# thanosDelatolas/eva-vos

Measured on AMD Instinct MI355X. Metric: frames/sec STCN mask-propagate 480p 1-obj, higher is better.
Workload: dtype f32; 1 GPU; DAVIS-17-val-shaped 480x854 (padded 480x864) single-object STCN propagate: fresh engine, interact(mask,0), T=66 frames/video, mem_freq=5, top_k=50; one video per step per GPU; videos_per_gpu=38, streams_per_gpu=4, key_lookahead=0, clips=8 distinct synthetic clips (one per pooled engine), weights=synthetic recipe seed 0 (no checkpoints offline)

## Files before the change

### eva_vos_amd/csrc/winograd4.hip

```cpp
#include <hip/hip_ext.h>

#include <cstdio>
#include <cstdlib>
#include <type_traits>

#include "wino_common.h"

namespace stcn {

typedef float f32x4 __attribute__((ext_vector_type(4)));
typedef float f32x16 __attribute__((ext_vector_type(16)));

#ifdef STCN_W4_CLOCK
__device__ unsigned long long g_w4_clock[2 * 8192];
#if STCN_W4_CLOCK == 2
#define W4_MFMA(a_, b_, c_) w4_fake_mfma(a_, b_, c_)
#endif
#endif
#ifndef W4_MFMA
#define W4_MFMA(a_, b_, c_) __builtin_amdgcn_mfma_f32_32x32x2f32(a_, b_, c_, 0, 0, 0)
#endif

static constexpr int W4T = 32;
static constexpr int W4N = 32;
static constexpr int W4W = 12;

#if defined(STCN_W4_CLOCK) && STCN_W4_CLOCK == 2
__device__ __forceinline__ f32x16 w4_fake_mfma(float a, float b, f32x16 c) {
#pragma unroll
    for (int e = 0; e < 16; ++e) asm volatile("v_fma_f32 %0, %1, %2, %0" : "+v"(c[e]) : "v"(a), "v"(b));
    return c;
}
#endif

__device__ __forceinline__ void bt6(const f32x4 &d0, const f32x4 &d1, const f32x4 &d2, const f32x4 &d3, const f32x4 &d4, const f32x4 &d5,
                                    f32x4 &o0, f32x4 &o1, f32x4 &o2, f32x4 &o3, f32x4 &o4, f32x4 &o5) {
    o0 = d0 * 1.265625f - d2 * 2.8125f + d4;
    const f32x4 e1 = d4 - d2 * 2.25f, f1 = d3 * 0.75f - d1 * 1.6875f;
    o1 = e1 + f1;
    o2 = e1 - f1;
    const f32x4 e2 = d4 - d2 * 0.5625f, f2 = d3 * 1.5f - d1 * 0.84375f;
    o3 = e2 + f2;
    o4 = e2 - f2;
    o5 = d1 * 1.265625f - d3 * 2.8125f + d5;
}

__global__ __launch_bounds__(256) void wino4_input_kernel(const float *__restrict__ x, unsigned x_bytes, long x_bs, int H, int W, int C,
                                                          int relu_in, int TH, int TW, int Mt, int Mt_pad, int cb_per_chunk,
                                                          int tile_lo, int tile_hi, float *__restrict__ V) {
    const long i = xcd_contiguous_block((int)blockIdx.x, (int)gridDim.x) * 256L + threadIdx.x;
    const int c16 = (int)(i & 7);
    const long tile = tile_lo + (i >> 3);
    if (tile >= tile_hi) return;
    const int KB = C / 8, NCB = C / 32;
    const int cb0 = blockIdx.y * cb_per_chunk, cb1 = min(NCB, cb0 + cb_per_chunk);
    const bool live = tile < Mt;
    const int tpi = TH * TW;
    const int b = live ? (int)(tile / tpi) : 0;
    const int r = live ? (int)(tile - (long)b * tpi) : 0;
    const int ty = r / TW, tx = r - ty * TW;
    const int y0 = 4 * ty - 1, x0 = 4 * tx - 1;
    unsigned long long ok = 0;
#pragma unroll
    for (int yy = 0; yy < 6; ++yy)
#pragma unroll
        for (int xx = 0; xx < 6; ++xx)
            if (live && (unsigned)(y0 + yy) < (unsigned)H && (unsigned)(x0 + xx) < (unsigned)W) ok |= 1ull << (yy * 6 + xx);
    const __amdgpu_buffer_rsrc_t rx = __builtin_amdgcn_make_buffer_rsrc(const_cast<float *>(x), 0, x_bytes, 0x00020000);
    const int xoff = (int)((b * x_bs + ((long)y0 * W + x0) * C + 4 * c16) * 4);
    const long ps = ((long)KB * Mt_pad) << 3;
    const float lo = relu_in ? 0.f : -__builtin_inff();
    for (int cb = cb0; cb < cb1; ++cb) {
        f32x4 t[6][6];
#pragma unroll
        for (int xx = 0; xx < 6; ++xx) {
            f32x4 d[6];
#pragma unroll
            for (int yy = 0; yy < 6; ++yy) {
                const unsigned vo = ((ok >> (yy * 6 + xx)) & 1ull) ? (unsigned)(xoff + ((yy * W + xx) * C + 32 * cb) * 4) : 0x80000000u;
                f32x4 v = __builtin_bit_cast(f32x4, __builtin_amdgcn_raw_buffer_load_b128(rx, vo, 0, 0));
                v.x = fmaxf(v.x, lo); v.y = fmaxf(v.y, lo); v.z = fmaxf(v.z, lo); v.w = fmaxf(v.w, lo);
                d[yy] = v;
            }
            bt6(d[0], d[1], d[2], d[3], d[4], d[5], t[0][xx], t[1][xx], t[2][xx], t[3][xx], t[4][xx], t[5][xx]);
        }
        const int kb = cb * 4 + (c16 >> 1);
        float *base = V + (((long)kb * Mt_pad + tile) << 3) + 4 * (c16 & 1);
#pragma unroll
        for (int xi = 0; xi < 6; ++xi) {
            f32x4 v[6];
            bt6(t[xi][0], t[xi][1], t[xi][2], t[xi][3], t[xi][4], t[xi][5], v[0], v[1], v[2], v[3], v[4], v[5]);
            float *dst = base + (long)(xi * 6) * ps;
#pragma unroll
            for (int nu = 0; nu < 6; ++nu) *reinterpret_cast<f32x4 *>(dst + nu * ps) = v[nu];
        }
    }
}

struct Wino4G {
    const float *V, *U;
    unsigned v_bytes, u_bytes;
    int Mt, Mt_pad, KB, N;
    int TH, TW, OH, OW, B, M;
    const float *bias, *res;
    long res_bs; int res_bmod;
    float *y; long y_bs;
    int relu_out;
    FastDiv fd_tpi, fd_tw, fd_tiles_n;
    int full_wg, pieces, kb_per_piece;
    float *partial;
    int tm0;
    int xb_m, xb_n, xb_cols;
};

template <int MB>
__global__ __launch_bounds__(64 * W4W) void wino4_gemm_kernel(const Wino4G p, const int tiles_n) {
    constexpr int PPW = 3, WT = W4T * MB;
    extern __shared__ __attribute__((aligned(16))) float smem[];
    int swz, piece = -1, kb0 = 0, kb1 = p.KB;
    if (MB == 1 && p.pieces > 1 && (int)blockIdx.x >= p.full_wg) {
        const int j = xcd_contiguous_block((int)blockIdx.x - p.full_wg, (int)gridDim.x - p.full_wg);
        const int rt = j / p.pieces;
        piece = j - rt * p.pieces;
        swz = p.full_wg + rt;
        kb0 = piece * p.kb_per_piece;
        kb1 = min(p.KB, kb0 + p.kb_per_piece);
    } else {
        swz = xcd_contiguous_block((int)blockIdx.x, MB == 1 && p.pieces > 1 ? p.full_wg : (int)gridDim.x);
    }
    int tm_l = fastdiv(swz, p.fd_tiles_n), tn = swz - tm_l * tiles_n;
    if (p.xb_m > 0 && piece < 0) {
        const int per = p.xb_m * p.xb_n, blk = swz / per, in = swz - blk * per;
        const int bm_i = blk / p.xb_cols, bn_i = blk - bm_i * p.xb_cols, im = in / p.xb_n;
        tm_l = bm_i * p.xb_m + im;
        tn = bn_i * p.xb_n + (in - im * p.xb_n);
    }
    const int tm = tm_l + p.tm0;
    const int t = threadIdx.x, lane = t & 63, l31 = lane & 31, h = lane >> 5;
    const int wave = __builtin_amdgcn_readfirstlane(t >> 6);
    const int pos0 = PPW * wave;

    const __amdgpu_buffer_rsrc_t rv = __builtin_amdgcn_make_buffer_rsrc(const_cast<float *>(p.V), 0, p.v_bytes, 0x00020000);
    const __amdgpu_buffer_rsrc_t ru = __builtin_amdgcn_make_buffer_rsrc(const_cast<float *>(p.U), 0, p.u_bytes, 0x00020000);
    const unsigned vl = (unsigned)(l31 * 32 + h * 16);
    unsigned sa0[PPW], sb0[PPW];
#pragma unroll
    for (int pi = 0; pi < PPW; ++pi) {
        sa0[pi] = (unsigned)((((long)(pos0 + pi) * p.KB + kb0) * p.Mt_pad + tm * WT) * 32);
        sb0[pi] = (unsigned)((((long)(pos0 + pi) * p.KB + kb0) * p.N + tn * W4N) * 32);
    }
    const unsigned sa = (unsigned)p.Mt_pad * 32u, sb = (unsigned)p.N * 32u;

    f32x16 acc[PPW][MB];
#pragma unroll
    for (int pi = 0; pi < PPW; ++pi)
#pragma unroll
        for (int bi = 0; bi < MB; ++bi)
#pragma unroll
            for (int e = 0; e < 16; ++e) acc[pi][bi][e] = 0.f;

    const int nk = kb1 - kb0;
    auto load1 = [&](int k, int pi, f32x4 (&fa)[MB], f32x4 &fb) {
        const unsigned oa = sa0[pi] + (unsigned)k * sa, ob = sb0[pi] + (unsigned)k * sb;
#pragma unroll
        for (int bi = 0; bi < MB; ++bi) fa[bi] = __builtin_bit_cast(f32x4, __builtin_amdgcn_raw_buffer_load_b128(rv, vl, oa + bi * 1024u, 0));
        fb = __builtin_bit_cast(f32x4, __builtin_amdgcn_raw_buffer_load_b128(ru, vl, ob, 0));
    };
    auto compute1 = [&](int pi, const f32x4 (&fa)[MB], const f32x4 &fb) {
#pragma unroll
        for (int j = 0; j < 4; ++j)
#pragma unroll
            for (int bi = 0; bi < MB; ++bi) acc[pi][bi] = W4_MFMA(fa[bi][j], fb[j], acc[pi][bi]);
    };
#ifdef STCN_W4_CLOCK
    unsigned long long ck_t0 = 0, ck_r0 = 0;
    if (wave == 0) {
        __builtin_amdgcn_sched_barrier(0);
        ck_t0 = __builtin_amdgcn_s_memtime();
        ck_r0 = __builtin_amdgcn_s_memrealtime();
        __builtin_amdgcn_s_waitcnt(0xC07F);
        __builtin_amdgcn_sched_barrier(0);
    }
#endif
    if (MB == 1) {
        f32x4 fa[3][PPW][MB], fb[3][PPW];
        auto load = [&](int k, int set) {
#pragma unroll
            for (int pi = 0; pi < PPW; ++pi) load1(k, pi, fa[set][pi], fb[set][pi]);
        };
        auto compute = [&](int set) {
#pragma unroll
            for (int j = 0; j < 4; ++j)
#pragma unroll
                for (int pi = 0; pi < PPW; ++pi)
#pragma unroll
                    for (int bi = 0; bi < MB; ++bi)
                        acc[pi][bi] = W4_MFMA(fa[set][pi][bi][j], fb[set][pi][j], acc[pi][bi]);
        };
        load(0, 0);
        load(min(1, nk - 1), 1);
        int k = 0;
        for (; k + 2 < nk; k += 3) {
            load(k + 2, 2);
            __builtin_amdgcn_sched_barrier(0);
            compute(0);
            __builtin_amdgcn_sched_barrier(0);
            load(min(k + 3, nk - 1), 0);
            __builtin_amdgcn_sched_barrier(0);
            compute(1);
            __builtin_amdgcn_sched_barrier(0);
            load(min(k + 4, nk - 1), 1);
            __builtin_amdgcn_sched_barrier(0);
            compute(2);
            __builtin_amdgcn_sched_barrier(0);
        }
        if (k < nk) compute(0);
        if (k + 1 < nk) compute(1);
    } else {
        f32x4 fa[2][PPW], fb[2][PPW];
        auto loadA = [&](int k, int bi, f32x4 (&d)[PPW]) {
#pragma unroll
            for (int pi = 0; pi < PPW; ++pi)
                d[pi] = __builtin_bit_cast(f32x4, __builtin_amdgcn_raw_buffer_load_b128(rv, vl, sa0[pi] + (unsigned)k * sa + bi * 1024u, 0));
        };
        auto loadB = [&](int k, f32x4 (&d)[PPW]) {
#pragma unroll
            for (int pi = 0; pi < PPW; ++pi)
                d[pi] = __builtin_bit_cast(f32x4, __builtin_amdgcn_raw_buffer_load_b128(ru, vl, sb0[pi] + (unsigned)k * sb, 0));
        };
        auto comp = [&](int bi, const f32x4 (&a)[PPW], const f32x4 (&bb)[PPW]) {
#pragma unroll
            for (int j = 0; j < 4; ++j)
#pragma unroll
                for (int pi = 0; pi < PPW; ++pi) acc[pi][bi] = W4_MFMA(a[pi][j], bb[pi][j], acc[pi][bi]);
        };
        loadB(0, fb[0]);
        loadA(0, 0, fa[0]);
        for (int k = 0; k < nk; k += 2) {
            const int k2 = min(k + 2, nk - 2);
            loadA(k, 1, fa[1]);
            __builtin_amdgcn_sched_barrier(0);
            comp(0, fa[0], fb[0]);
            __builtin_amdgcn_sched_barrier(0);
            loadB(k + 1, fb[1]);
            loadA(k + 1, 0, fa[0]);
            __builtin_amdgcn_sched_barrier(0);
            comp(1, fa[1], fb[0]);
            __builtin_amdgcn_sched_barrier(0);
            loadA(k + 1, 1, fa[1]);
            __builtin_amdgcn_sched_barrier(0);
            comp(0, fa[0], fb[1]);
            __builtin_amdgcn_sched_barrier(0);
            loadB(k2, fb[0]);
            loadA(k2, 0, fa[0]);
            __builtin_amdgcn_sched_barrier(0);
            comp(1, fa[1], fb[1]);
            __builtin_amdgcn_sched_barrier(0);
        }
    }
#ifdef STCN_W4_CLOCK
    if (wave == 0) {
        __builtin_amdgcn_sched_barrier(0);
        const unsigned long long ck_t1 = __builtin_amdgcn_s_memtime(), ck_r1 = __builtin_amdgcn_s_memrealtime();
        __builtin_amdgcn_s_waitcnt(0xC07F);
        __builtin_amdgcn_sched_barrier(0);
        if (lane == 0 && blockIdx.x < 8192) { g_w4_clock[2 * blockIdx.x] = ck_t1 - ck_t0; g_w4_clock[2 * blockIdx.x + 1] = ck_r1 - ck_r0; }
    }
#endif
    const int chq = t & 7, tl = (t >> 3) & 31;
    const int jh = __builtin_amdgcn_readfirstlane(t >> 8);
    const int tpi = p.TH * p.TW, ohw = p.OH * p.OW;
    const int n = tn * W4N + 4 * chq;
    const bool kpiece = MB == 1 && piece >= 0;
    const float lo = p.relu_out ? 0.f : -__builtin_inff();
    const __amdgpu_buffer_rsrc_t rres = __builtin_amdgcn_make_buffer_rsrc(const_cast<float *>(p.res ? p.res : p.y), 0, -1, 0x00020000);
    const __amdgpu_buffer_rsrc_t ry = __builtin_amdgcn_make_buffer_rsrc(p.y, 0, -1, 0x00020000);
    const unsigned y_bs = (unsigned)(p.y_bs ? p.y_bs : (long)ohw * p.N);
#pragma unroll
    for (int half = 0; half < MB; ++half) {
        int toff = 32 * half + tl;
        asm volatile("" : "+v"(toff));
        const long gt = (long)tm * WT + toff;
        const bool work = jh < 2 && gt < p.Mt;
        const int gtc = (int)min(gt, (long)p.Mt - 1);
        const int b = fastdiv(gtc, p.fd_tpi);
        const int rr = gtc - b * tpi;
        const int ty = fastdiv(rr, p.fd_tw), tx = rr - ty * p.TW;
        unsigned prow[4], pcol[2];
#pragma unroll
        for (int i2 = 0; i2 < 4; ++i2) prow[i2] = (unsigned)(min(4 * ty + i2, p.OH - 1) * p.OW * p.N) * 4u;
#pragma unroll
        for (int j = 0; j < 2; ++j) pcol[j] = (unsigned)(min(4 * tx + 2 * jh + j, p.OW - 1) * p.N + n) * 4u;
        if (half) __syncthreads();
#pragma unroll
        for (int pi = 0; pi < PPW; ++pi)
#pragma unroll
            for (int r = 0; r < 16; ++r)
                smem[((pos0 + pi) * W4T + (r & 3) + 8 * (r >> 2) + 4 * h) * W4N + l31] = acc[pi][half][r];
        f32x4 yv[2][4], bv = {0.f, 0.f, 0.f, 0.f};
        if (p.bias && !kpiece) {
            int nb = n;
            asm volatile("" : "+v"(nb));
            bv = *reinterpret_cast<const f32x4 *>(p.bias + nb);
        }
        if (p.res && !kpiece && jh < 2) {
            const unsigned rb = (unsigned)(p.res_bmod ? b % p.res_bmod : b) * (unsigned)p.res_bs * 4u;
#pragma unroll
            for (int j = 0; j < 2; ++j)
#pragma unroll
                for (int i2 = 0; i2 < 4; ++i2)
                    yv[j][i2] = __builtin_bit_cast(f32x4, __builtin_amdgcn_raw_buffer_load_b128(rres, rb + prow[i2] + pcol[j], 0, 0));
        } else {
#pragma unroll
            for (int j = 0; j < 2; ++j)
#pragma unroll
                for (int i2 = 0; i2 < 4; ++i2) yv[j][i2] = f32x4{0.f, 0.f, 0.f, 0.f};
        }
        __syncthreads();
        if (!work) continue;
        auto zrow = [&](int xi, auto JH, f32x4 (&zr)[2]) {
            f32x4 m[6];
            int ro4 = (xi * 6 * W4T + tl) * (W4N / 4) + chq;
            asm volatile("" : "+v"(ro4));
#pragma unroll
            for (int nu = 0; nu < 6; ++nu) m[nu] = reinterpret_cast<const f32x4 *>(smem)[ro4 + nu * W4T * (W4N / 4)];
            if (decltype(JH)::value == 0) {
                zr[0] = m[0] + (m[1] + m[2]) + (m[3] + m[4]);
                zr[1] = (m[1] - m[2]) * 0.75f + (m[3] - m[4]) * 1.5f;
            } else {
                zr[0] = (m[1] + m[2]) * 0.5625f + (m[3] + m[4]) * 2.25f;
                zr[1] = (m[1] - m[2]) * 0.421875f + (m[3] - m[4]) * 3.375f + m[5];
            }
        };
        auto columns = [&](auto JH) {
            f32x4 za[2];
#pragma unroll
            for (int j = 0; j < 2; ++j)
#pragma unroll
                for (int i2 = 0; i2 < 4; ++i2) yv[j][i2] += bv;
            zrow(0, JH, za);
#pragma unroll
            for (int j = 0; j < 2; ++j) yv[j][0] += za[j];
            constexpr float c1[4] = {0.75f, -0.75f, 1.5f, -1.5f}, c2[4] = {0.5625f, 0.5625f, 2.25f, 2.25f},
                            c3[4] = {0.421875f, -0.421875f, 3.375f, -3.375f};
#pragma unroll
            for (int xi = 1; xi < 5; ++xi) {
                __builtin_amdgcn_sched_barrier(0);
                zrow(xi, JH, za);
#pragma unroll
                for (int j = 0; j < 2; ++j) {
                    yv[j][0] += za[j];
                    yv[j][1] += za[j] * c1[xi - 1];
                    yv[j][2] += za[j] * c2[xi - 1];
                    yv[j][3] += za[j] * c3[xi - 1];
                }
            }
            __builtin_amdgcn_sched_barrier(0);
            zrow(5, JH, za);
#pragma unroll
            for (int j = 0; j < 2; ++j) yv[j][3] += za[j];
        };
        if (jh == 0) columns(std::integral_constant<int, 0>{});
        else columns(std::integral_constant<int, 1>{});
        if (kpiece) {
            float *dst = p.partial + (((long)(swz - p.full_wg) * p.pieces + piece) * W4T + tl) * (16 * W4N) + 4 * chq;
#pragma unroll
            for (int j = 0; j < 2; ++j)
#pragma unroll
                for (int i2 = 0; i2 < 4; ++i2) *reinterpret_cast<f32x4 *>(dst + (i2 * 4 + 2 * jh + j) * W4N) = yv[j][i2];
            continue;
        }
        const unsigned yb = (unsigned)b * y_bs * 4u;
#pragma unroll
        for (int j = 0; j < 2; ++j)
#pragma unroll
            for (int i2 = 0; i2 < 4; ++i2) {
#pragma unroll
                for (int c = 0; c < 4; ++c) yv[j][i2][c] = fmaxf(yv[j][i2][c], lo);
                const bool ok = 4 * tx + 2 * jh + j < p.OW && 4 * ty + i2 < p.OH;
                __builtin_amdgcn_raw_buffer_store_b128(__builtin_bit_cast(__attribute__((__vector_size__(4 * sizeof(unsigned)))) unsigned, yv[j][i2]), ry,
                                                       ok ? yb + prow[i2] + pcol[j] : 0xFFFFFFFFu, 0, 0);
            }
    }
}

__global__ __launch_bounds__(256) void wino4_reduce_kernel(const Wino4G p, const int tiles_n) {
    const int rt = blockIdx.x >> 6, swz = p.full_wg + rt;
    const int tm = fastdiv(swz, p.fd_tiles_n), tn = swz - tm * tiles_n;
    const int n_l = threadIdx.x & 31;
    const int e = ((blockIdx.x & 63) << 3) + (threadIdx.x >> 5);
    const int tl = e >> 4, px = e & 15;
    const int n = tn * W4N + n_l;
    const long gt = (long)tm * W4T + tl;
    if (gt >= p.Mt) return;
    const int tpi = p.TH * p.TW, ohw = p.OH * p.OW;
    const int b = fastdiv((int)gt, p.fd_tpi);
    const int rr = (int)(gt - (long)b * tpi);
    const int ty = fastdiv(rr, p.fd_tw), tx = rr - ty * p.TW;
    const int oh = 4 * ty + (px >> 2), ow = 4 * tx + (px & 3);
    if (oh >= p.OH || ow >= p.OW) return;
    const float *src = p.partial + ((long)rt * p.pieces * W4T * 16 + e) * W4N + n_l;
    float pv[8];
#pragma unroll
    for (int s2 = 0; s2 < 8; ++s2) pv[s2] = src[(long)min(s2, p.pieces - 1) * (W4T * 16 * W4N)];
    const long po = ((long)oh * p.OW + ow) * p.N + n;
    const float rv = p.res ? p.res[(long)(p.res_bmod ? b % p.res_bmod : b) * p.res_bs + po] : 0.f;
    float v = 0.f;
#pragma unroll
    for (int s2 = 0; s2 < 8; ++s2) v += s2 < p.pieces ? pv[s2] : 0.f;
    v += (p.bias ? p.bias[n] : 0.f) + rv;
    p.y[(p.y_bs ? (long)b * p.y_bs : (long)b * ohw * p.N) + po] = fmaxf(v, p.relu_out ? 0.f : -__builtin_inff());
}

int wino4_mode() {
    static const int m = env_int("STCN_WINO4", 1);
    return m;
}

static KPieces wino4_small_pieces(int grid, int KB) {
    static const bool on = env_on("STCN_WINO4_SMALL");
    const int cus = device_cus();
    if (!on || grid * 2 > cus) return {1, KB};
    return k_pieces(cus / grid, KB, 8, 8);
}

static W4Plan wino4_gemm_plan(const ConvP &p, const WinoGeom &ge, size_t slab_floats) {
    static const int mb_env = env_int("STCN_WINO4_MB", 0);
    static const bool tail_on = env_on("STCN_WINO4_TAIL");
    const int cus = device_cus(), KB = ge.KB;
    W4Plan pl{};
    pl.tiles_n = p.N / W4N;
    pl.mb = mb_env == 1 || mb_env == 2 ? mb_env : ((ge.Mt_pad / (2 * W4T)) * pl.tiles_n >= 200 ? 2 : 1);
    pl.tiles_m = ge.Mt_pad / (W4T * pl.mb);
    pl.grid = pl.tiles_m * pl.tiles_n;
    pl.full_wg = pl.grid; pl.pieces = 1; pl.per = KB;
    const bool may_split = tail_on && pl.mb == 1 && p.partial;
    if (may_split) {
        const int full = pl.grid / cus * cus, rem = pl.grid - full;
        if (full >= cus && rem > 0 && rem <= cus / 2) {
            const KPieces kp = k_pieces(cus / rem, KB, 8, 8);
            if (kp.pieces > 1 && (size_t)rem * kp.pieces * W4T * 16 * W4N <= slab_floats) {
                pl.full_wg = full; pl.pieces = kp.pieces; pl.per = kp.per;
                pl.grid = full + rem * kp.pieces;
            }
        }
    }
    const int wg32 = (ge.Mt_pad / W4T) * pl.tiles_n;
    const KPieces small = wino4_small_pieces(wg32, KB);
    pl.judge_wg = wg32 * small.pieces;
    if (may_split && pl.pieces == 1 && small.pieces > 1 && (size_t)pl.grid * small.pieces * W4T * 16 * W4N <= slab_floats) {
        pl.full_wg = 0; pl.pieces = small.pieces; pl.per = small.per;
        pl.grid *= small.pieces;
    }
    pl.chunks = 1; pl.tm_per_chunk = pl.tiles_m;
    const long chunk_bytes = (long)p.kn.wino4_chunk_mb << 20;
    const long vbytes = 36L * p.Cin * ge.Mt_pad * 4;
    if (pl.mb == 2 && chunk_bytes > 0 && vbytes > chunk_bytes * 3 / 2) {
        const int rounds = (pl.grid + cus - 1) / cus;
        const int n = (int)((vbytes + chunk_bytes - 1) / chunk_bytes);
        const int rpc = (rounds + n - 1) / n;
        int tmpc = rpc * cus / pl.tiles_n;
        tmpc = tmpc < 1 ? 1 : tmpc;
        if (tmpc < pl.tiles_m && (pl.tiles_m + tmpc - 1) / tmpc <= W4_MAX_CHUNKS) { pl.tm_per_chunk = tmpc; pl.chunks = (pl.tiles_m + tmpc - 1) / tmpc; }
    }
    return pl;
}

bool wino4_plan(const ConvP &p, int min_wg, size_t v_cap, size_t slab_floats, ConvPlan &cp) {
    if (!wino4_mode() || !p.wino4_u || p.KH != 3 || p.KW != 3 || p.stride != 1 || p.x1) return false;
    if (p.Cin % 32 || p.Cin < W4_MIN_CIN || p.N % W4N || p.bs0 == 0) return false;
    const WinoGeom ge = wino_geom(p, 4, 2 * W4T);
    if (!wino_extents_ok(p, 36, ge.Mt_pad)) return false;
    const W4Plan w4 = wino4_gemm_plan(p, ge, slab_floats);
    if (wino4_mode() < 2 && w4.judge_wg < min_wg) return false;
    const size_t need = (size_t)36 * p.Cin * ge.Mt_pad;
    if (need > v_cap) return false;
    cp.family = CONV_WINO4;
    cp.geo = ge; cp.w4 = w4;
    cp.v_floats = need;
    cp.n_in = cp.n_gemm = w4.chunks; cp.reduce = w4.pieces > 1;
    cp.fl_exec = 2.0 * (double)need * p.N;
    return true;
}

void wino4_launch(const ConvP &p, const ConvPlan &cp, float *V, hipStream_t s, hipEvent_t *const *ev_in, hipEvent_t *const *ev_gemm,
                  hipEvent_t *ev_red) {
    const W4Plan &pl = cp.w4;
    const WinoGeom &ge = cp.geo;
    const int tiles_n = pl.tiles_n, mb = pl.mb, tiles_m = pl.tiles_m;
    Wino4G g{};
    wino_fill_desc(g, p, ge, 36, V, p.wino4_u, tiles_n);
    g.full_wg = pl.full_wg; g.pieces = pl.pieces; g.kb_per_piece = pl.per; g.partial = p.partial;
    g.xb_m = g.xb_n = g.xb_cols = 0;
    {
        const int rows = pl.full_wg / tiles_n;
        if (pl.chunks == 1 && pl.full_wg % 8 == 0 && rows * tiles_n == pl.full_wg && tiles_n >= 8) {
            const int per = pl.full_wg / 8;
            int best = 0, best_sum = per % tiles_n == 0 ? per / tiles_n + tiles_n : rows + tiles_n;
            for (int bn = 2; bn <= tiles_n; ++bn) {
                if (per % bn || tiles_n % bn) continue;
                const int bm = per / bn;
                if (bm < 1 || rows % bm || (rows / bm) * (tiles_n / bn) != 8) continue;
                if (bm + bn < best_sum) { best_sum = bm + bn; best = bn; }
            }
            if (best && best != tiles_n) { g.xb_n = best; g.xb_m = per / best; g.xb_cols = tiles_n / best; }
        }
    }
    const size_t lds = (size_t)36 * W4T * W4N * sizeof(float);
    for (int c = 0; c < pl.chunks; ++c) {
        const int tm_lo = c * pl.tm_per_chunk, tm_hi = tm_lo + pl.tm_per_chunk < tiles_m ? tm_lo + pl.tm_per_chunk : tiles_m;
        const int tile_lo = tm_lo * W4T * mb, tile_hi = pl.chunks == 1 ? ge.Mt_pad : tm_hi * W4T * mb;
        hipEvent_t *ei = ev_in ? ev_in[c] : nullptr, *eg = ev_gemm ? ev_gemm[c] : nullptr;
        const WinoInGrid ig = wino_input_grid(tile_hi - tile_lo, p.Cin);
        launch(wino4_input_kernel, dim3(ig.gx, ig.chunks), dim3(256), 0, s, ei, p.x0, p.x0_bytes, p.bs0, p.H, p.W, p.Cin, p.relu_in, ge.TH, ge.TW,
               ge.Mt, ge.Mt_pad, ig.per, tile_lo, tile_hi, V);
        g.tm0 = tm_lo;
        if (mb == 2) {
            const int grid = (tm_hi - tm_lo) * tiles_n;
            launch(wino4_gemm_kernel<2>, dim3(grid), dim3(64 * W4W), lds, s, eg, g, tiles_n);
        } else {
            launch(wino4_gemm_kernel<1>, dim3(pl.grid), dim3(64 * W4W), lds, s, eg, g, tiles_n);
            if (g.pieces > 1) launch(wino4_reduce_kernel, dim3((tiles_m * tiles_n - g.full_wg) * 64), dim3(256), 0, s, ev_red, g, tiles_n);
        }
    }
}

void wino4_transform_weights(const float *w, int N, int Cin, int Kp, float *U) {
    static const double G[6][3] = {{64.0 / 81, 0, 0},
                                   {-128.0 / 243, -32.0 / 81, -8.0 / 27},
                                   {-128.0 / 243, 32.0 / 81, -8.0 / 27},
                                   {32.0 / 243, 16.0 / 81, 8.0 / 27},
                                   {32.0 / 243, -16.0 / 81, 8.0 / 27},
                                   {0, 0, 1}};
    wino_transform_weights_with(G, w, N, Cin, Kp, U);
}

#ifdef STCN_W4_CLOCK
extern "C" int stcn_debug_w4_clock(unsigned long long *host_out, int n_pairs) {
    return hipMemcpyFromSymbol(host_out, HIP_SYMBOL(g_w4_clock), (size_t)2 * (n_pairs < 8192 ? n_pairs : 8192) * sizeof(unsigned long long)) == hipSuccess ? 0 : 1;
}
#endif

}
```

Before: 830.3 frames/s.

## Restructure Winograd F(4,3) GEMM prologue and epilogue for fewer instructions

```diff
diff --git a/eva_vos_amd/csrc/winograd4.hip b/eva_vos_amd/csrc/winograd4.hip
--- a/eva_vos_amd/csrc/winograd4.hip
+++ b/eva_vos_amd/csrc/winograd4.hip
@@ -12,10 +12,21 @@
 typedef float f32x16 __attribute__((ext_vector_type(16)));
 
 #ifdef STCN_W4_CLOCK
-__device__ unsigned long long g_w4_clock[2 * 8192];
+static constexpr int W4_CK_REC = 8;
+__device__ unsigned long long g_w4_clock[W4_CK_REC * 8192];
+#define W4_STAMP(dst_, wait_)                                  \
+    if (wave == 0) {                                           \
+        __builtin_amdgcn_sched_barrier(0);                     \
+        __builtin_amdgcn_s_waitcnt(wait_);                     \
+        dst_ = __builtin_amdgcn_s_memtime();                   \
+        __builtin_amdgcn_s_waitcnt(0xC07F);                    \
+        __builtin_amdgcn_sched_barrier(0);                     \
+    }
 #if STCN_W4_CLOCK == 2
 #define W4_MFMA(a_, b_, c_) w4_fake_mfma(a_, b_, c_)
 #endif
+#else
+#define W4_STAMP(dst_, wait_)
 #endif
 #ifndef W4_MFMA
 #define W4_MFMA(a_, b_, c_) __builtin_amdgcn_mfma_f32_32x32x2f32(a_, b_, c_, 0, 0, 0)
@@ -32,6 +43,8 @@
     return c;
 }
 #endif
+
+__device__ __forceinline__ f32x4 fma4(const f32x4 &a, float c, const f32x4 &b) { return __builtin_elementwise_fma(a, f32x4{c, c, c, c}, b); }
 
 __device__ __forceinline__ void bt6(const f32x4 &d0, const f32x4 &d1, const f32x4 &d2, const f32x4 &d3, const f32x4 &d4, const f32x4 &d5,
                                     f32x4 &o0, f32x4 &o1, f32x4 &o2, f32x4 &o3, f32x4 &o4, f32x4 &o5) {
@@ -118,6 +131,15 @@
     constexpr int PPW = 3, WT = W4T * MB;
     extern __shared__ __attribute__((aligned(16))) float smem[];
     int swz, piece = -1, kb0 = 0, kb1 = p.KB;
+#ifdef STCN_W4_CLOCK
+    unsigned long long ck_e = 0, ck_w[2] = {0, 0}, ck_s[2] = {0, 0};
+    if (__builtin_amdgcn_readfirstlane(threadIdx.x >> 6) == 0) {
+        __builtin_amdgcn_sched_barrier(0);
+        ck_e = __builtin_amdgcn_s_memtime();
+        __builtin_amdgcn_s_waitcnt(0xC07F);
+        __builtin_amdgcn_sched_barrier(0);
+    }
+#endif
     if (MB == 1 && p.pieces > 1 && (int)blockIdx.x >= p.full_wg) {
         const int j = xcd_contiguous_block((int)blockIdx.x - p.full_wg, (int)gridDim.x - p.full_wg);
         const int rt = j / p.pieces;
@@ -152,28 +174,13 @@
     const unsigned sa = (unsigned)p.Mt_pad * 32u, sb = (unsigned)p.N * 32u;
 
     f32x16 acc[PPW][MB];
-#pragma unroll
-    for (int pi = 0; pi < PPW; ++pi)
-#pragma unroll
-        for (int bi = 0; bi < MB; ++bi)
-#pragma unroll
-            for (int e = 0; e < 16; ++e) acc[pi][bi][e] = 0.f;
+    const f32x16 zero16 = {0.f, 0.f, 0.f, 0.f, 0.f, 0.f, 0.f, 0.f, 0.f, 0.f, 0.f, 0.f, 0.f, 0.f, 0.f, 0.f};
+    constexpr std::true_type first_c{};
+    constexpr std::false_type later_c{};
 
     const int nk = kb1 - kb0;
-    auto load1 = [&](int k, int pi, f32x4 (&fa)[MB], f32x4 &fb) {
-        const unsigned oa = sa0[pi] + (unsigned)k * sa, ob = sb0[pi] + (unsigned)k * sb;
-#pragma unroll
-        for (int bi = 0; bi < MB; ++bi) fa[bi] = __builtin_bit_cast(f32x4, __builtin_amdgcn_raw_buffer_load_b128(rv, vl, oa + bi * 1024u, 0));
-        fb = __builtin_bit_cast(f32x4, __builtin_amdgcn_raw_buffer_load_b128(ru, vl, ob, 0));
-    };
-    auto compute1 = [&](int pi, const f32x4 (&fa)[MB], const f32x4 &fb) {
-#pragma unroll
-        for (int j = 0; j < 4; ++j)
-#pragma unroll
-            for (int bi = 0; bi < MB; ++bi) acc[pi][bi] = W4_MFMA(fa[bi][j], fb[j], acc[pi][bi]);
-    };
 #ifdef STCN_W4_CLOCK
-    unsigned long long ck_t0 = 0, ck_r0 = 0;
+    unsigned long long ck_t0 = 0, ck_r0 = 0, ck_l1 = 0, ck_dr = 0;
     if (wave == 0) {
         __builtin_amdgcn_sched_barrier(0);
         ck_t0 = __builtin_amdgcn_s_memtime();
@@ -183,39 +190,50 @@
     }
 #endif
     if (MB == 1) {
-        f32x4 fa[3][PPW][MB], fb[3][PPW];
+        f32x4 fa[3][PPW], fb[3][PPW];
         auto load = [&](int k, int set) {
-#pragma unroll
-            for (int pi = 0; pi < PPW; ++pi) load1(k, pi, fa[set][pi], fb[set][pi]);
-        };
-        auto compute = [&](int set) {
+            const unsigned ka = (unsigned)k * sa, kb = (unsigned)k * sb;
+#pragma unroll
+            for (int pi = 0; pi < PPW; ++pi) {
+                fa[set][pi] = __builtin_bit_cast(f32x4, __builtin_amdgcn_raw_buffer_load_b128(rv, vl, sa0[pi] + ka, 0));
+                fb[set][pi] = __builtin_bit_cast(f32x4, __builtin_amdgcn_raw_buffer_load_b128(ru, vl, sb0[pi] + kb, 0));
+            }
+        };
+        auto compute = [&](int set, auto FIRST) {
 #pragma unroll
             for (int j = 0; j < 4; ++j)
 #pragma unroll
-                for (int pi = 0; pi < PPW; ++pi)
-#pragma unroll
-                    for (int bi = 0; bi < MB; ++bi)
-                        acc[pi][bi] = W4_MFMA(fa[set][pi][bi][j], fb[set][pi][j], acc[pi][bi]);
+                for (int pi = 0; pi < PPW; ++pi) {
+                    if (decltype(FIRST)::value && j == 0) acc[pi][0] = W4_MFMA(fa[set][pi][j], fb[set][pi][j], zero16);
+                    else acc[pi][0] = W4_MFMA(fa[set][pi][j], fb[set][pi][j], acc[pi][0]);
+                }
+        };
+        auto body = [&](int k, auto FIRST) {
+            load(k + 2, 2);
+            __builtin_amdgcn_sched_barrier(0);
+            compute(0, FIRST);
+            __builtin_amdgcn_sched_barrier(0);
+            load(min(k + 3, nk - 1), 0);
+            __builtin_amdgcn_sched_barrier(0);
+            compute(1, later_c);
+            __builtin_amdgcn_sched_barrier(0);
+            load(min(k + 4, nk - 1), 1);
+            __builtin_amdgcn_sched_barrier(0);
+            compute(2, later_c);
+            __builtin_amdgcn_sched_barrier(0);
         };
         load(0, 0);
         load(min(1, nk - 1), 1);
-        int k = 0;
-        for (; k + 2 < nk; k += 3) {
-            load(k + 2, 2);
-            __builtin_amdgcn_sched_barrier(0);
-            compute(0);
-            __builtin_amdgcn_sched_barrier(0);
-            load(min(k + 3, nk - 1), 0);
-            __builtin_amdgcn_sched_barrier(0);
-            compute(1);
-            __builtin_amdgcn_sched_barrier(0);
-            load(min(k + 4, nk - 1), 1);
-            __builtin_amdgcn_sched_barrier(0);
-            compute(2);
-            __builtin_amdgcn_sched_barrier(0);
-        }
-        if (k < nk) compute(0);
-        if (k + 1 < nk) compute(1);
+        if (nk > 2) {
+            body(0, first_c);
+            int k = 3;
+            for (; k + 2 < nk; k += 3) body(k, later_c);
+            if (k < nk) compute(0, later_c);
+            if (k + 1 < nk) compute(1, later_c);
+        } else {
+            compute(0, first_c);
+            if (nk > 1) compute(1, later_c);
+        }
     } else {
         f32x4 fa[2][PPW], fb[2][PPW];
         auto loadA = [&](int k, int bi, f32x4 (&d)[PPW]) {
@@ -228,35 +246,40 @@
             for (int pi = 0; pi < PPW; ++pi)
                 d[pi] = __builtin_bit_cast(f32x4, __builtin_amdgcn_raw_buffer_load_b128(ru, vl, sb0[pi] + (unsigned)k * sb, 0));
         };
-        auto comp = [&](int bi, const f32x4 (&a)[PPW], const f32x4 (&bb)[PPW]) {
+        auto comp = [&](int bi, const f32x4 (&a)[PPW], const f32x4 (&bb)[PPW], auto FIRST) {
 #pragma unroll
             for (int j = 0; j < 4; ++j)
 #pragma unroll
-                for (int pi = 0; pi < PPW; ++pi) acc[pi][bi] = W4_MFMA(a[pi][j], bb[pi][j], acc[pi][bi]);
+                for (int pi = 0; pi < PPW; ++pi) {
+                    if (decltype(FIRST)::value && j == 0) acc[pi][bi] = W4_MFMA(a[pi][j], bb[pi][j], zero16);
+                    else acc[pi][bi] = W4_MFMA(a[pi][j], bb[pi][j], acc[pi][bi]);
+                }
+        };
+        auto body = [&](int k, auto FIRST) {
+            const int k2 = min(k + 2, nk - 2);
+            loadA(k, 1, fa[1]);
+            __builtin_amdgcn_sched_barrier(0);
+            comp(0, fa[0], fb[0], FIRST);
+            __builtin_amdgcn_sched_barrier(0);
+            loadB(k + 1, fb[1]);
+            loadA(k + 1, 0, fa[0]);
+            __builtin_amdgcn_sched_barrier(0);
+            comp(1, fa[1], fb[0], FIRST);
+            __builtin_amdgcn_sched_barrier(0);
+            loadA(k + 1, 1, fa[1]);
+            __builtin_amdgcn_sched_barrier(0);
+            comp(0, fa[0], fb[1], later_c);
+            __builtin_amdgcn_sched_barrier(0);
+            loadB(k2, fb[0]);
+            loadA(k2, 0, fa[0]);
+            __builtin_amdgcn_sched_barrier(0);
+            comp(1, fa[1], fb[1], later_c);
+            __builtin_amdgcn_sched_barrier(0);
         };
         loadB(0, fb[0]);
         loadA(0, 0, fa[0]);
-        for (int k = 0; k < nk; k += 2) {
-            const int k2 = min(k + 2, nk - 2);
-            loadA(k, 1, fa[1]);
-            __builtin_amdgcn_sched_barrier(0);
-            comp(0, fa[0], fb[0]);
-            __builtin_amdgcn_sched_barrier(0);
-            loadB(k + 1, fb[1]);
-            loadA(k + 1, 0, fa[0]);
-            __builtin_amdgcn_sched_barrier(0);
-            comp(1, fa[1], fb[0]);
-            __builtin_amdgcn_sched_barrier(0);
-            loadA(k + 1, 1, fa[1]);
-            __builtin_amdgcn_sched_barrier(0);
-            comp(0, fa[0], fb[1]);
-            __builtin_amdgcn_sched_barrier(0);
-            loadB(k2, fb[0]);
-            loadA(k2, 0, fa[0]);
-            __builtin_amdgcn_sched_barrier(0);
-            comp(1, fa[1], fb[1]);
-            __builtin_amdgcn_sched_barrier(0);
-        }
+        body(0, first_c);
+        for (int k = 2; k < nk; k += 2) body(k, later_c);
     }
 #ifdef STCN_W4_CLOCK
     if (wave == 0) {
@@ -264,124 +287,144 @@
         const unsigned long long ck_t1 = __builtin_amdgcn_s_memtime(), ck_r1 = __builtin_amdgcn_s_memrealtime();
         __builtin_amdgcn_s_waitcnt(0xC07F);
         __builtin_amdgcn_sched_barrier(0);
-        if (lane == 0 && blockIdx.x < 8192) { g_w4_clock[2 * blockIdx.x] = ck_t1 - ck_t0; g_w4_clock[2 * blockIdx.x + 1] = ck_r1 - ck_r0; }
+        ck_l1 = ck_t1; ck_dr = ck_r1 - ck_r0;
     }
 #endif
     const int chq = t & 7, tl = (t >> 3) & 31;
     const int jh = __builtin_amdgcn_readfirstlane(t >> 8);
-    const int tpi = p.TH * p.TW, ohw = p.OH * p.OW;
-    const int n = tn * W4N + 4 * chq;
-    const bool kpiece = MB == 1 && piece >= 0;
-    const float lo = p.relu_out ? 0.f : -__builtin_inff();
-    const __amdgpu_buffer_rsrc_t rres = __builtin_amdgcn_make_buffer_rsrc(const_cast<float *>(p.res ? p.res : p.y), 0, -1, 0x00020000);
-    const __amdgpu_buffer_rsrc_t ry = __builtin_amdgcn_make_buffer_rsrc(p.y, 0, -1, 0x00020000);
-    const unsigned y_bs = (unsigned)(p.y_bs ? p.y_bs : (long)ohw * p.N);
-#pragma unroll
-    for (int half = 0; half < MB; ++half) {
-        int toff = 32 * half + tl;
-        asm volatile("" : "+v"(toff));
-        const long gt = (long)tm * WT + toff;
-        const bool work = jh < 2 && gt < p.Mt;
-        const int gtc = (int)min(gt, (long)p.Mt - 1);
-        const int b = fastdiv(gtc, p.fd_tpi);
-        const int rr = gtc - b * tpi;
-        const int ty = fastdiv(rr, p.fd_tw), tx = rr - ty * p.TW;
-        unsigned prow[4], pcol[2];
-#pragma unroll
-        for (int i2 = 0; i2 < 4; ++i2) prow[i2] = (unsigned)(min(4 * ty + i2, p.OH - 1) * p.OW * p.N) * 4u;
-#pragma unroll
-        for (int j = 0; j < 2; ++j) pcol[j] = (unsigned)(min(4 * tx + 2 * jh + j, p.OW - 1) * p.N + n) * 4u;
-        if (half) __syncthreads();
-#pragma unroll
-        for (int pi = 0; pi < PPW; ++pi)
-#pragma unroll
-            for (int r = 0; r < 16; ++r)
-                smem[((pos0 + pi) * W4T + (r & 3) + 8 * (r >> 2) + 4 * h) * W4N + l31] = acc[pi][half][r];
-        f32x4 yv[2][4], bv = {0.f, 0.f, 0.f, 0.f};
-        if (p.bias && !kpiece) {
-            int nb = n;
-            asm volatile("" : "+v"(nb));
-            bv = *reinterpret_cast<const f32x4 *>(p.bias + nb);
-        }
-        if (p.res && !kpiece && jh < 2) {
-            const unsigned rb = (unsigned)(p.res_bmod ? b % p.res_bmod : b) * (unsigned)p.res_bs * 4u;
+    auto epilogue = [&](auto KP) {
+        constexpr bool kp = decltype(KP)::value;
+#pragma unroll
+        for (int half = 0; half < MB; ++half) {
+            if (half) __syncthreads();
+#pragma unroll
+            for (int pi = 0; pi < PPW; ++pi)
+#pragma unroll
+                for (int r = 0; r < 16; ++r)
+                    smem[((pos0 + pi) * W4T + (r & 3) + 8 * (r >> 2) + 4 * h) * W4N + l31] = acc[pi][half][r];
+            W4_STAMP(ck_w[half], 0xC07F);
+            int toff = 32 * half + tl;
+            asm volatile("" : "+v"(toff));
+            const int tlp = toff - 32 * half;
+            const long gt = (long)tm * WT + toff;
+            const bool work = jh < 2 && gt < p.Mt;
+            const int n = tn * W4N + 4 * chq;
+            int b = 0, ty = 0, tx = 0;
+            unsigned prow[4], pcol[2];
+            f32x4 yv[2][4], bv = {0.f, 0.f, 0.f, 0.f};
 #pragma unroll
             for (int j = 0; j < 2; ++j)
 #pragma unroll
-                for (int i2 = 0; i2 < 4; ++i2)
-                    yv[j][i2] = __builtin_bit_cast(f32x4, __builtin_amdgcn_raw_buffer_load_b128(rres, rb + prow[i2] + pcol[j], 0, 0));
-        } else {
-#pragma unroll
-            for (int j = 0; j < 2; ++j)
-#pragma unroll
                 for (int i2 = 0; i2 < 4; ++i2) yv[j][i2] = f32x4{0.f, 0.f, 0.f, 0.f};
-        }
-        __syncthreads();
-        if (!work) continue;
-        auto zrow = [&](int xi, auto JH, f32x4 (&zr)[2]) {
-            f32x4 m[6];
-            int ro4 = (xi * 6 * W4T + tl) * (W4N / 4) + chq;
-            asm volatile("" : "+v"(ro4));
-#pragma unroll
-            for (int nu = 0; nu < 6; ++nu) m[nu] = reinterpret_cast<const f32x4 *>(smem)[ro4 + nu * W4T * (W4N / 4)];
-            if (decltype(JH)::value == 0) {
-                zr[0] = m[0] + (m[1] + m[2]) + (m[3] + m[4]);
-                zr[1] = (m[1] - m[2]) * 0.75f + (m[3] - m[4]) * 1.5f;
-            } else {
-                zr[0] = (m[1] + m[2]) * 0.5625f + (m[3] + m[4]) * 2.25f;
-                zr[1] = (m[1] - m[2]) * 0.421875f + (m[3] - m[4]) * 3.375f + m[5];
-            }
-        };
-        auto columns = [&](auto JH) {
-            f32x4 za[2];
-#pragma unroll
-            for (int j = 0; j < 2; ++j)
-#pragma unroll
-                for (int i2 = 0; i2 < 4; ++i2) yv[j][i2] += bv;
-            zrow(0, JH, za);
-#pragma unroll
-            for (int j = 0; j < 2; ++j) yv[j][0] += za[j];
-            constexpr float c1[4] = {0.75f, -0.75f, 1.5f, -1.5f}, c2[4] = {0.5625f, 0.5625f, 2.25f, 2.25f},
-                            c3[4] = {0.421875f, -0.421875f, 3.375f, -3.375f};
-#pragma unroll
-            for (int xi = 1; xi < 5; ++xi) {
-                __builtin_amdgcn_sched_barrier(0);
-                zrow(xi, JH, za);
-#pragma unroll
-                for (int j = 0; j < 2; ++j) {
-                    yv[j][0] += za[j];
-                    yv[j][1] += za[j] * c1[xi - 1];
-                    yv[j][2] += za[j] * c2[xi - 1];
-                    yv[j][3] += za[j] * c3[xi - 1];
+            if (!kp) {
+                const int tpi = p.TH * p.TW;
+                const int gtc = (int)min(gt, (long)p.Mt - 1);
+                b = fastdiv(gtc, p.fd_tpi);
+                const int rr = gtc - b * tpi;
+                ty = fastdiv(rr, p.fd_tw);
+                tx = rr - ty * p.TW;
+#pragma unroll
+                for (int i2 = 0; i2 < 4; ++i2) prow[i2] = (unsigned)(min(4 * ty + i2, p.OH - 1) * p.OW * p.N) * 4u;
+#pragma unroll
+                for (int j = 0; j < 2; ++j) pcol[j] = (unsigned)(min(4 * tx + 2 * jh + j, p.OW - 1) * p.N + n) * 4u;
+                if (p.bias) bv = *reinterpret_cast<const f32x4 *>(p.bias + n);
+                if (p.res && jh < 2) {
+                    const __amdgpu_buffer_rsrc_t rres = __builtin_amdgcn_make_buffer_rsrc(const_cast<float *>(p.res), 0, -1, 0x00020000);
+                    const unsigned rb = (unsigned)(p.res_bmod ? b % p.res_bmod : b) * (unsigned)p.res_bs * 4u;
+#pragma unroll
+                    for (int j = 0; j < 2; ++j)
+#pragma unroll
+                        for (int i2 = 0; i2 < 4; ++i2)
+                            yv[j][i2] = __builtin_bit_cast(f32x4, __builtin_amdgcn_raw_buffer_load_b128(rres, rb + prow[i2] + pcol[j], 0, 0));
                 }
             }
-            __builtin_amdgcn_sched_barrier(0);
-            zrow(5, JH, za);
-#pragma unroll
-            for (int j = 0; j < 2; ++j) yv[j][3] += za[j];
-        };
-        if (jh == 0) columns(std::integral_constant<int, 0>{});
-        else columns(std::integral_constant<int, 1>{});
-        if (kpiece) {
-            float *dst = p.partial + (((long)(swz - p.full_wg) * p.pieces + piece) * W4T + tl) * (16 * W4N) + 4 * chq;
-#pragma unroll
-            for (int j = 0; j < 2; ++j)
-#pragma unroll
-                for (int i2 = 0; i2 < 4; ++i2) *reinterpret_cast<f32x4 *>(dst + (i2 * 4 + 2 * jh + j) * W4N) = yv[j][i2];
-            continue;
-        }
-        const unsigned yb = (unsigned)b * y_bs * 4u;
-#pragma unroll
-        for (int j = 0; j < 2; ++j)
-#pragma unroll
-            for (int i2 = 0; i2 < 4; ++i2) {
-#pragma unroll
-                for (int c = 0; c < 4; ++c) yv[j][i2][c] = fmaxf(yv[j][i2][c], lo);
-                const bool ok = 4 * tx + 2 * jh + j < p.OW && 4 * ty + i2 < p.OH;
-                __builtin_amdgcn_raw_buffer_store_b128(__builtin_bit_cast(__attribute__((__vector_size__(4 * sizeof(unsigned)))) unsigned, yv[j][i2]), ry,
-                                                       ok ? yb + prow[i2] + pcol[j] : 0xFFFFFFFFu, 0, 0);
+            __syncthreads();
+            if (work) {
+                const int rpb = MB == 2 && half == 0 ? 1 : 3;
+                const f32x4 *sm4 = reinterpret_cast<const f32x4 *>(smem) + (tlp * (W4N / 4) + chq);
+                auto columns = [&](auto JH) {
+                    constexpr int jhc = decltype(JH)::value;
+                    constexpr float c1[4] = {0.75f, -0.75f, 1.5f, -1.5f}, c2[4] = {0.5625f, 0.5625f, 2.25f, 2.25f},
+                                    c3[4] = {0.421875f, -0.421875f, 3.375f, -3.375f};
+#pragma unroll
+                    for (int j = 0; j < 2; ++j)
+#pragma unroll
+                        for (int i2 = 0; i2 < 4; ++i2) yv[j][i2] += bv;
+#pragma unroll
+                    for (int batch = 0; batch < 6 / rpb; ++batch) {
+                        f32x4 m[3][6];
+#pragma unroll
+                        for (int r = 0; r < rpb; ++r)
+#pragma unroll
+                            for (int nu = (jhc == 0 ? 0 : 1); nu < (jhc == 0 ? 5 : 6); ++nu)
+                                m[r][nu] = sm4[((rpb * batch + r) * 6 + nu) * W4T * (W4N / 4)];
+                        __builtin_amdgcn_sched_barrier(0);
+#pragma unroll
+                        for (int r = 0; r < rpb; ++r) {
+                            const int xi = rpb * batch + r;
+                            f32x4 za[2];
+                            if (jhc == 0) {
+                                za[0] = m[r][0] + (m[r][1] + m[r][2]) + (m[r][3] + m[r][4]);
+                                za[1] = fma4(m[r][1] - m[r][2], 0.75f, (m[r][3] - m[r][4]) * 1.5f);
+                            } else {
+                                za[0] = fma4(m[r][1] + m[r][2], 0.5625f, (m[r][3] + m[r][4]) * 2.25f);
+                                za[1] = fma4(m[r][1] - m[r][2], 0.421875f, (m[r][3] - m[r][4]) * 3.375f) + m[r][5];
+                            }
+#pragma unroll
+                            for (int j = 0; j < 2; ++j) {
+                                if (xi == 0) yv[j][0] += za[j];
+                                else if (xi == 5) yv[j][3] += za[j];
+                                else {
+                                    yv[j][0] += za[j];
+                                    yv[j][1] = fma4(za[j], c1[xi - 1], yv[j][1]);
+                                    yv[j][2] = fma4(za[j], c2[xi - 1], yv[j][2]);
+                                    yv[j][3] = fma4(za[j], c3[xi - 1], yv[j][3]);
+                                }
+                            }
+                        }
+                        __builtin_amdgcn_sched_barrier(0);
+                    }
+                };
+                if (jh == 0) columns(std::integral_constant<int, 0>{});
+                else columns(std::integral_constant<int, 1>{});
+                if (kp) {
+                    float *dst = p.partial + (((long)(swz - p.full_wg) * p.pieces + piece) * W4T + tlp) * (16 * W4N) + 4 * chq;
+#pragma unroll
+                    for (int j = 0; j < 2; ++j)
+#pragma unroll
+                        for (int i2 = 0; i2 < 4; ++i2) *reinterpret_cast<f32x4 *>(dst + (i2 * 4 + 2 * jh + j) * W4N) = yv[j][i2];
+                } else {
+                    const __amdgpu_buffer_rsrc_t ry = __builtin_amdgcn_make_buffer_rsrc(p.y, 0, -1, 0x00020000);
+                    const float lo = p.relu_out ? 0.f : -__builtin_inff();
+                    const unsigned y_bs = (unsigned)(p.y_bs ? p.y_bs : (long)p.OH * p.OW * p.N);
+                    const unsigned yb = (unsigned)b * y_bs * 4u;
+#pragma unroll
+                    for (int j = 0; j < 2; ++j)
+#pragma unroll
+                        for (int i2 = 0; i2 < 4; ++i2) {
+#pragma unroll
+                            for (int c = 0; c < 4; ++c) yv[j][i2][c] = fmaxf(yv[j][i2][c], lo);
+                            const bool ok = 4 * tx + 2 * jh + j < p.OW && 4 * ty + i2 < p.OH;
+                            __builtin_amdgcn_raw_buffer_store_b128(__builtin_bit_cast(__attribute__((__vector_size__(4 * sizeof(unsigned)))) unsigned, yv[j][i2]), ry,
+                                                                   ok ? yb + prow[i2] + pcol[j] : 0xFFFFFFFFu, 0, 0);
+                        }
+                }
             }
-    }
+            if (half + 1 < MB) { W4_STAMP(ck_s[half], 0xC07F); } else { W4_STAMP(ck_s[half], 0); }
+        }
+    };
+    const bool kpiece = MB == 1 && piece >= 0;
+    if (kpiece) epilogue(std::true_type{});
+    else epilogue(std::false_type{});
+#ifdef STCN_W4_CLOCK
+    if (wave == 0 && lane == 0 && blockIdx.x < 8192) {
+        unsigned long long *o = g_w4_clock + (size_t)W4_CK_REC * blockIdx.x;
+        o[0] = ck_t0 - ck_e; o[1] = ck_l1 - ck_t0; o[2] = ck_dr;
+        o[3] = ck_w[0] - ck_l1; o[4] = ck_s[0] - ck_w[0];
+        o[5] = MB == 2 ? ck_w[MB - 1] - ck_s[0] : 0; o[6] = MB == 2 ? ck_s[MB - 1] - ck_w[MB - 1] : 0;
+        o[7] = kpiece ? 1 : 0;
+    }
+#endif
 }
 
 __global__ __launch_bounds__(256) void wino4_reduce_kernel(const Wino4G p, const int tiles_n) {
@@ -536,9 +579,9 @@
 }
 
 #ifdef STCN_W4_CLOCK
-extern "C" int stcn_debug_w4_clock(unsigned long long *host_out, int n_pairs) {
-    return hipMemcpyFromSymbol(host_out, HIP_SYMBOL(g_w4_clock), (size_t)2 * (n_pairs < 8192 ? n_pairs : 8192) * sizeof(unsigned long long)) == hipSuccess ? 0 : 1;
-}
-#endif
-
-}
+extern "C" int stcn_debug_w4_clock(unsigned long long *host_out, int n_records) {
+    return hipMemcpyFromSymbol(host_out, HIP_SYMBOL(g_w4_clock), (size_t)W4_CK_REC * (n_records < 8192 ? n_records : 8192) * sizeof(unsigned long long)) == hipSuccess ? 0 : 1;
+}
+#endif
+
+}
```

After: 825.2 frames/s. About the same (-0.6%).
